# qurAI-amsterdam/SuperResolution_aniso_MRI

Measured on AMD Instinct MI355X. Metric: training slices/sec (ae_combined, 160x160, latent=128), higher is better.
Workload: dtype f32; 1 GPU; ACDC synthetic 12x(3x1x160x160) triplets, ae_combined latent=128 depth=32 scales=2, MSE synthesis loss (BASELINE configs[1]); global_batch_triplets=12, parallelism=dp1, init=reference Initializer, seed 892372, random weights, launch=captured HIP graph replay

## Files before the change

### superresolution_aniso_mri_amd/csrc/conv_wgrad_wino.hip

```cpp
#include <stdio.h>
#include <stdlib.h>

#include <type_traits>
#include <utility>

#include "aesr_kernels.h"

constexpr int WW_OOB = 0x70000000;
typedef float f32x2 __attribute__((ext_vector_type(2)));

template <int... I, class F>
__device__ __forceinline__ void ww_for(std::integer_sequence<int, I...>, F&& f) {
    (f(std::integral_constant<int, I>{}), ...);
}
template <int N, class F>
__device__ __forceinline__ void ww_rep(F&& f) { ww_for(std::make_integer_sequence<int, N>{}, f); }

__device__ __forceinline__ void ww_dma(__amdgpu_buffer_rsrc_t rs, float* lds_wave_base, int byte_off) {
    __builtin_amdgcn_raw_ptr_buffer_load_lds(rs, (__attribute__((address_space(3))) void*)lds_wave_base, 16, byte_off, 0, 0, 0);
}

#define WW_PK(dst, a, b, mods)                                                          \
    do {                                                                                \
        f32x2& d_ = dst;                                                                \
        const f32x2 a_ = a, b_ = b;                                                     \
        asm volatile("v_pk_add_f32 %0, %1, %2 " mods : "=v"(d_) : "v"(a_), "v"(b_));    \
    } while (0)
#define WW_M_ADD ""
#define WW_M_SUB "neg_lo:[0,1] neg_hi:[0,1]"
#define WW_M_T01 "op_sel:[0,0] op_sel_hi:[1,0] neg_lo:[0,1] neg_hi:[0,0]"
#define WW_M_T23 "op_sel:[1,0] op_sel_hi:[1,1] neg_lo:[1,0] neg_hi:[0,1]"
#define WW_M_LL "op_sel:[0,0] op_sel_hi:[0,0] neg_lo:[0,0] neg_hi:[0,1]"
#define WW_M_HH "op_sel:[1,1] op_sel_hi:[1,1] neg_lo:[0,0] neg_hi:[0,1]"
#define WW_M_SELF "op_sel:[0,1] op_sel_hi:[0,1] neg_lo:[0,0] neg_hi:[0,1]"

struct WwTile {
    int n, ty, tx;
};

template <int TH, int TW, bool STAMP>
__global__ __launch_bounds__(256, 1) void conv_wgrad_wino_f32(WgradArgs a) {
    constexpr int CIT = 32, COT = 32;
    static_assert((TH == 16 && TW == 8) || (TH == 8 && TW == 16), "tiles: 8 k-steps, rows of whole 8-pixel DMA segments");
    constexpr int PH = TH + 2, PWL = TW == 8 ? 16 : 32, TWL = TW;
    constexpr int XFL = PH * PWL * 32, DFL = TH * TWL * 32;
    constexpr int KPR = TW >> 3;
    constexpr int SPR = PWL / 8, SPRD = TW / 8;
    constexpr int NXS = PH * SPR / 4, NDS = TH * SPRD / 4;
    constexpr int RXS = 4 / SPR, RDS = 4 / SPRD;
    static_assert(2 * (XFL + DFL) * 4 <= 160 * 1024 && (PH * SPR) % 4 == 0 && (TH * SPRD) % 4 == 0, "LDS / segment split");

    extern __shared__ __attribute__((aligned(16))) float lds[];
    const int tid = threadIdx.x, lane = tid & 63;
    const int wave = __builtin_amdgcn_readfirstlane(tid >> 6);
    const int l15 = lane & 15, g = lane >> 4;
    const int nci = a.CinP / CIT, nchunks = nci * (a.CoutP / COT);
    int chunk, split;
    if ((a.S & 7) == 0) {
        const int xcd = blockIdx.x & 7, local = blockIdx.x >> 3;
        chunk = local % nchunks;
        split = (local / nchunks) * 8 + xcd;
    } else {
        chunk = blockIdx.x % nchunks;
        split = blockIdx.x / nchunks;
    }
    const int ciy = chunk % nci, coz = chunk / nci;
    const int ci0 = ciy * CIT, co0 = coz * COT;
    float* const ldsX0 = lds;
    float* const ldsD0 = lds + 2 * XFL;
    const bool do_bias = ciy == 0;

    const int sh = a.x_up2 ? 1 : 0;
    const int xH = a.H >> sh, xW = a.W >> sh;
    const int ximg = xH * xW * a.Cin * 4, dimg = a.H * a.W * a.Cout * 4;
    const int xrow = xW * a.Cin * 4, drow = a.W * a.Cout * 4;
    const int sgx = wave % SPR, rx0 = wave / SPR, sgd = wave % SPRD, rd0 = wave / SPRD;
    const int pxl = lane >> 3, pos = lane & 7;
    const int quad = pos ^ (((pxl >> 1) & 1) << 2);
    const int pcx = 8 * sgx + pxl, pcd = 8 * sgd + pxl;
    const int lcx = (((pcx - sh) >> sh) * a.Cin + ci0 + 4 * quad) * 4;
    const int lcd = (pcd * a.Cout + co0 + 4 * quad) * 4;
    const int tpi = a.tiles_y * a.tiles_x;
    const int dS_n = a.S / tpi, dS_r = a.S - dS_n * tpi, dS_ty = dS_r / a.tiles_x, dS_tx = dS_r - dS_ty * a.tiles_x;
    auto advance = [&](WwTile t) {
        t.tx += dS_tx;
        if (t.tx >= a.tiles_x) { t.tx -= a.tiles_x; ++t.ty; }
        t.ty += dS_ty;
        if (t.ty >= a.tiles_y) { t.ty -= a.tiles_y; ++t.n; }
        t.n += dS_n;
        return t;
    };
    auto fetch = [&](const WwTile& t, int buf) {
        const bool valid = t.n < a.N;
        const int n = valid ? t.n : 0, y0 = t.ty * TH, x0 = t.tx * TW;
        const __amdgpu_buffer_rsrc_t rs_x = __builtin_amdgcn_make_buffer_rsrc((void*)((const char*)a.x + (size_t)n * ximg), 0, valid ? ximg : 0, 0x00020000);
        const __amdgpu_buffer_rsrc_t rs_d = __builtin_amdgcn_make_buffer_rsrc((void*)((const char*)a.dy + (size_t)n * dimg), 0, valid ? dimg : 0, 0x00020000);
        const unsigned gxx = (unsigned)(x0 - 1 + pcx), gxd = (unsigned)(x0 + pcd);
        const int offx = (pcx < TW + 2 && gxx < (unsigned)a.W) ? lcx + ((x0 >> sh) - 1 + sh) * a.Cin * 4 : WW_OOB;
        const int offd = gxd < (unsigned)a.W ? lcd + x0 * a.Cout * 4 : WW_OOB;
        const int r0 = y0 - 1 + rx0;
        int ux = (r0 >> sh) * xrow;
        const int step_odd = sh == 0 ? RXS * xrow : RXS == 2 ? xrow : (r0 & 1) * xrow;
        const int step_even = sh == 0 ? RXS * xrow : RXS == 2 ? xrow : xrow - step_odd;
        float* const xdst = ldsX0 + buf * XFL + (rx0 * PWL + 8 * sgx) * 32;
        int uxk[NXS];
        ww_rep<NXS>([&](auto Kc) {
            constexpr int k = decltype(Kc)::value;
            if constexpr (k > 0) ux += (k & 1) ? step_odd : step_even;
            uxk[k] = ux;
        });
        if (pcx < TW + 2) {
            ww_rep<NXS>([&](auto Kc) {
                constexpr int k = decltype(Kc)::value;
                ww_dma(rs_x, xdst + k * RXS * PWL * 32, offx + uxk[k]);
            });
        }
        int ud = (y0 + rd0) * drow;
        float* const ddst = ldsD0 + buf * DFL + (rd0 * TWL + 8 * sgd) * 32;
        ww_rep<NDS>([&](auto Kc) {
            constexpr int k = decltype(Kc)::value;
            if constexpr (k > 0) ud += RDS * drow;
            ww_dma(rs_d, ddst + k * RDS * TWL * 32, offd + ud);
        });
    };

    f32x4 acc[16][2][2];
#pragma unroll
    for (int x = 0; x < 16; ++x)
#pragma unroll
        for (int i = 0; i < 2; ++i)
#pragma unroll
            for (int o = 0; o < 2; ++o) acc[x][i][o] = (f32x4){0.f, 0.f, 0.f, 0.f};
    float accb[2] = {0.f, 0.f};

    const int sw = (g & 1) << 2;
    const int chA = (((l15 >> 2) ^ sw) << 2) + (l15 & 3);
    const int chB = (((l15 >> 2) ^ sw ^ 4) << 2) + (l15 & 3);
    const unsigned lds0 = (unsigned)(unsigned long long)lds;
    unsigned lx[2][4], ld[2][2];
#pragma unroll
    for (int i = 0; i < 2; ++i) {
#pragma unroll
        for (int c = 0; c < 4; ++c) lx[i][c] = lds0 + (unsigned)(((2 * g + c) * 32 + ((c < 2 ? chA : chB) ^ (i ? 16 : 0))) * 4);
#pragma unroll
        for (int e = 0; e < 2; ++e) ld[i][e] = lds0 + (unsigned)((2 * XFL + (2 * g + e) * 32 + (chA ^ (i ? 16 : 0))) * 4);
    }

    f32x2 Vp[2][2][2][4], Mp[2][2][8];
    f32x2 P[2][4][2];
    auto op_read = [&](int xu, int du, int nb) {
        ww_rep<8>([&](auto Kc) {
            constexpr int i = decltype(Kc)::value >> 2, c = decltype(Kc)::value & 3;
            const unsigned ad = lx[i][c] + (unsigned)(xu * 4);
            f32x2 &p0_ = P[i][c][0], &p1_ = P[i][c][1];
            asm volatile("ds_read2st64_b32 %0, %2 offset0:%3 offset1:%4\n\tds_read2st64_b32 %1, %2 offset0:%5 offset1:%6"
                         : "=&v"(p0_), "=&v"(p1_) : "v"(ad), "n"(0), "n"(PWL / 2), "n"(PWL), "n"(3 * PWL / 2) : "memory");
        });
        ww_rep<4>([&](auto Kc) {
            constexpr int o = decltype(Kc)::value >> 1, e = decltype(Kc)::value & 1;
            const unsigned ad = ld[o][e] + (unsigned)(du * 4);
            f32x2& y_ = Mp[nb][o][e];
            asm volatile("ds_read2st64_b32 %0, %1 offset0:0 offset1:%2" : "=&v"(y_) : "v"(ad), "n"(TWL / 2) : "memory");
        });
    };
    auto op_transform = [&](int nb) {
        asm volatile("s_waitcnt lgkmcnt(0)" ::: "memory");
        ww_rep<2>([&](auto Ic) {
            constexpr int i = decltype(Ic)::value;
            f32x2 T[2][4];
            ww_rep<4>([&](auto Cc) {
                constexpr int c = decltype(Cc)::value;
                WW_PK(T[0][c], P[i][c][0], P[i][c][1], WW_M_T01);
                WW_PK(T[1][c], P[i][c][0], P[i][c][1], WW_M_T23);
            });
            ww_rep<2>([&](auto Sc) {
                constexpr int s_ = decltype(Sc)::value;
                WW_PK(Vp[nb][i][s_][0], T[s_][0], T[s_][2], WW_M_SUB);
                WW_PK(Vp[nb][i][s_][1], T[s_][1], T[s_][2], WW_M_ADD);
                WW_PK(Vp[nb][i][s_][2], T[s_][2], T[s_][1], WW_M_SUB);
                WW_PK(Vp[nb][i][s_][3], T[s_][1], T[s_][3], WW_M_SUB);
            });
        });
        ww_rep<2>([&](auto Oc) {
            constexpr int o = decltype(Oc)::value;
            WW_PK(Mp[nb][o][2], Mp[nb][o][0], Mp[nb][o][0], WW_M_SELF);
            WW_PK(Mp[nb][o][3], Mp[nb][o][1], Mp[nb][o][1], WW_M_SELF);
            WW_PK(Mp[nb][o][4], Mp[nb][o][0], Mp[nb][o][1], WW_M_LL);
            WW_PK(Mp[nb][o][7], Mp[nb][o][0], Mp[nb][o][1], WW_M_HH);
            WW_PK(Mp[nb][o][5], Mp[nb][o][2], Mp[nb][o][3], WW_M_LL);
            WW_PK(Mp[nb][o][6], Mp[nb][o][2], Mp[nb][o][3], WW_M_HH);
            accb[o] += Mp[nb][o][5][0];
        });
    };
    auto mfmas = [&](auto Q0c, auto Nc, int cb) {
        ww_rep<decltype(Nc)::value>([&](auto Dc) {
            constexpr int q = decltype(Q0c)::value + decltype(Dc)::value, x = q >> 2, i = (q >> 1) & 1, o = q & 1;
            constexpr int r = x >> 2, k = x & 3;
            constexpr int mi = k == 0 ? (r == 0 || r == 3 ? 0 : 2) : k == 3 ? (r == 0 || r == 3 ? 1 : 3) : 4 + r;
            constexpr int mh = k == 0 || k == 3 ? (r >= 2 ? 1 : 0) : k - 1;
            f32x4& acc_ = acc[x][i][o];
            const float va_ = Vp[cb][i][r >> 1][k][r & 1], vb_ = Mp[cb][o][mi][mh];
            asm volatile("v_mfma_f32_16x16x4_f32 %0, %1, %2, %0" : "+a"(acc_) : "v"(va_), "v"(vb_));
        });
    };
    auto step_xu = [&](int j, int buf) { const int ks = wave + 4 * j, tyl = ks / KPR, kx = ks - tyl * KPR; return buf * XFL + ((2 * tyl) * PWL + 8 * kx) * 32; };
    auto step_du = [&](int j, int buf) { const int ks = wave + 4 * j, tyl = ks / KPR, kx = ks - tyl * KPR; return buf * DFL + ((2 * tyl) * TWL + 8 * kx) * 32; };
    using C0 = std::integral_constant<int, 0>;
    using C16 = std::integral_constant<int, 16>;
    using C32 = std::integral_constant<int, 32>;

    long long tph[3] = {0, 0, 0}, tq = 0;
#define WW_STAMP(k)                                                   \
    if constexpr (STAMP) {                                            \
        const long long t_ = (long long)__builtin_amdgcn_s_memtime(); \
        tph[k] += t_ - tq;                                            \
        tq = t_;                                                      \
    }
    if constexpr (STAMP) tq = (long long)__builtin_amdgcn_s_memtime();

    WwTile t0, t1, t2;
    {
        t0.n = split / tpi;
        const int rem = split - t0.n * tpi;
        t0.ty = rem / a.tiles_x;
        t0.tx = rem - t0.ty * a.tiles_x;
        if (split >= a.ntiles) t0.n = a.N;
    }
    t1 = advance(t0);
    t2 = advance(t1);
    fetch(t0, 0);
    fetch(t1, 1);
    asm volatile("s_waitcnt vmcnt(0)" ::: "memory");
    __syncthreads();
    int buf = 0;
    op_read(step_xu(0, 0), step_du(0, 0), 0);
    op_transform(0);
    WW_STAMP(2)
    if (t0.n < a.N) do {
        __builtin_amdgcn_sched_barrier(0);
        op_read(step_xu(1, buf), step_du(1, buf), 1);
        mfmas(C0{}, C16{}, 0);
        op_transform(1);
        mfmas(C16{}, std::integral_constant<int, 48>{}, 0);
        __builtin_amdgcn_sched_barrier(0);
        WW_STAMP(0)
        asm volatile("s_waitcnt vmcnt(0) lgkmcnt(0)" ::: "memory");
        __syncthreads();
        WW_STAMP(1)
        __builtin_amdgcn_sched_barrier(0);
        op_read(step_xu(0, buf ^ 1), step_du(0, buf ^ 1), 0);
        mfmas(C0{}, C16{}, 1);
        __builtin_amdgcn_sched_barrier(0);
        fetch(t2, buf);
        __builtin_amdgcn_sched_barrier(0);
        mfmas(C16{}, C16{}, 1);
        op_transform(0);
        mfmas(C32{}, C32{}, 1);
        __builtin_amdgcn_sched_barrier(0);
        t0 = t1;
        t1 = t2;
        t2 = advance(t2);
        buf ^= 1;
    } while (t0.n < a.N);
    WW_STAMP(0)
    asm volatile("s_waitcnt vmcnt(0) lgkmcnt(0)" ::: "memory");
    __syncthreads();
    if (STAMP && lane == 0)
        for (int k = 0; k < 3; ++k) a.dbgbuf[(blockIdx.x * 4 + wave) * 3 + k] = (float)tph[k];

    f32x4 dg[9][2][2];
#pragma unroll
    for (int i = 0; i < 2; ++i)
#pragma unroll
        for (int o = 0; o < 2; ++o) {
            f32x4 R[3][4];
#pragma unroll
            for (int j = 0; j < 4; ++j) {
                const f32x4 u0_ = acc[0 + j][i][o], u1 = acc[4 + j][i][o], u2 = acc[8 + j][i][o], u3 = -acc[12 + j][i][o];
                const f32x4 s = j == 3 ? (f32x4){-1.f, -1.f, -1.f, -1.f} : (f32x4){1.f, 1.f, 1.f, 1.f};
                R[0][j] = s * (u0_ + 0.5f * (u1 + u2));
                R[1][j] = s * (0.5f * (u1 - u2));
                R[2][j] = s * (0.5f * (u1 + u2) + u3);
            }
#pragma unroll
            for (int r = 0; r < 3; ++r) {
                dg[r * 3 + 0][i][o] = R[r][0] + 0.5f * (R[r][1] + R[r][2]);
                dg[r * 3 + 1][i][o] = 0.5f * (R[r][1] - R[r][2]);
                dg[r * 3 + 2][i][o] = 0.5f * (R[r][1] + R[r][2]) + R[r][3];
            }
        }
#pragma unroll
    for (int o = 0; o < 2; ++o) {
        accb[o] += __shfl_xor(accb[o], 16, 64);
        accb[o] += __shfl_xor(accb[o], 32, 64);
    }
    f32x4* ex = (f32x4*)lds;
    float* exb = lds + 4 * 36 * 64 * 4;
#pragma unroll
    for (int t = 0; t < 9; ++t)
#pragma unroll
        for (int i = 0; i < 2; ++i)
#pragma unroll
            for (int o = 0; o < 2; ++o) ex[(wave * 36 + (t * 4 + i * 2 + o)) * 64 + lane] = dg[t][i][o];
    if (g == 0) {
        exb[wave * 32 + l15] = accb[0];
        exb[wave * 32 + 16 + l15] = accb[1];
    }
    __syncthreads();
    const size_t plane = (size_t)a.CinP * a.CoutP;
    float* sl = a.slab + (size_t)split * 10 * plane;
#pragma unroll
    for (int q = 0; q < 9; ++q) {
        const int blk = wave * 9 + q;
        const int t = blk >> 2, i = (blk >> 1) & 1, o = blk & 1;
        f32x4 v = ex[(0 * 36 + blk) * 64 + lane];
#pragma unroll
        for (int w = 1; w < 4; ++w) v += ex[(w * 36 + blk) * 64 + lane];
        const int co = co0 + o * 16 + l15;
#pragma unroll
        for (int e = 0; e < 4; ++e) {
            const int ci = ci0 + i * 16 + g * 4 + e;
            sl[t * plane + (size_t)ci * a.CoutP + co] = v[e];
        }
    }
    if (wave == 0 && do_bias && g == 0) {
#pragma unroll
        for (int o = 0; o < 2; ++o) {
            float bsum = exb[0 * 32 + o * 16 + l15];
#pragma unroll
            for (int w = 1; w < 4; ++w) bsum += exb[w * 32 + o * 16 + l15];
            sl[9 * plane + co0 + o * 16 + l15] = bsum;
        }
    }
}

size_t aesr_wgrad_wino_lds_bytes(int TH, int TW) {
    const size_t xfl = (size_t)(TH + 2) * (TW == 8 ? 16 : 32) * 32, dfl = (size_t)TH * TW * 32;
    const size_t bufs = 2 * (xfl + dfl) * sizeof(float);
    const size_t exch = ((size_t)4 * 36 * 64 * 4 + 4 * 32) * sizeof(float);
    return bufs > exch ? bufs : exch;
}

bool aesr_wgrad_wino_tile_ok(int TH, int TW) { return (TH == 16 && TW == 8) || (TH == 8 && TW == 16); }

template <int TH, int TW>
static int launch_wgrad_wino(const WgradArgs& a, hipStream_t st) {
    const size_t shmem = aesr_wgrad_wino_lds_bytes(TH, TW);
    static bool attr_set[AESR_MAX_DEVICES] = {}, attr_set_dbg[AESR_MAX_DEVICES] = {};
    if (int e = aesr_lds_opt_in((const void*)conv_wgrad_wino_f32<TH, TW, false>, "conv_wgrad_wino_f32", attr_set)) return e;
    (void)aesr_lds_opt_in((const void*)conv_wgrad_wino_f32<TH, TW, true>, "conv_wgrad_wino_f32", attr_set_dbg);
    dim3 grid(a.S * (a.CinP / 32) * (a.CoutP / 32));
    if (getenv("AESR_WGRAD_WINO_DBG") && grid.x <= 4096) {
        static float* dbuf = nullptr;
        if (!dbuf) (void)hipMalloc(&dbuf, 4096 * 4 * 3 * sizeof(float));
        WgradArgs b = a;
        b.dbgbuf = dbuf;
        hipLaunchKernelGGL((conv_wgrad_wino_f32<TH, TW, true>), grid, dim3(256), shmem, st, b);
        (void)hipStreamSynchronize(st);
        static float host[4096 * 4 * 3];
        (void)hipMemcpy(host, dbuf, (size_t)grid.x * 4 * 3 * sizeof(float), hipMemcpyDeviceToHost);
        double s3[3] = {0, 0, 0};
        for (unsigned i = 0; i < grid.x * 4; ++i) for (int k = 0; k < 3; ++k) s3[k] += host[i * 3 + k];
        const double visits = (double)((a.ntiles + a.S - 1) / a.S);
        const int nks = (TH >> 1) * (TW >> 3);
        fprintf(stderr, "[wgrad-wino stamps] grid=%u tile %dx%d S=%d (%.0f visits, %d k-steps = %d MFMA cycles per wave and visit) per visit, cycles: "
                "k-step loop %.0f | barrier %.0f || fill %.0f\n", grid.x, TH, TW, a.S, visits, nks, nks / 4 * 64 * 32,
                s3[0] / grid.x / 4 / visits, s3[1] / grid.x / 4 / visits, s3[2] / grid.x / 4);
        return AESR_OK;
    }
    hipLaunchKernelGGL((conv_wgrad_wino_f32<TH, TW, false>), grid, dim3(256), shmem, st, a);
    AESR_LAUNCH_CHECK("conv_wgrad_wino_f32");
    return AESR_OK;
}

int aesr_launch_conv_wgrad_wino(const WgradArgs& a, hipStream_t st) {
    if ((size_t)a.H * a.W * a.Cin * 4 >= (size_t)0x10000000 || (size_t)a.H * a.W * a.Cout * 4 >= (size_t)0x10000000) {
        aesr_set_error("conv_wgrad_wino: images of 256 MB or more need 64-bit lane offsets (not built)");
        return AESR_ERR_UNSUPPORTED;
    }
    if (a.x_up2 && ((a.H | a.W) & 1)) {
        aesr_set_error("conv_wgrad_wino: the folded Upsample(x2) needs even convolution sizes (got %dx%d)", a.H, a.W);
        return AESR_ERR_ARG;
    }
    if (!aesr_wgrad_wino_tile_ok(a.TH, a.TW) || a.pad != 1 || a.Ho != a.H || a.Wo != a.W) {
        aesr_set_error("conv_wgrad_wino: tile %dx%d is not 16x8 or 8x16 (or not 3x3 / padding 1)", a.TH, a.TW);
        return AESR_ERR_ARG;
    }
    if (a.CinP % 32 != 0 || a.CoutP % 32 != 0 || a.Cin != a.CinP || a.Cout != a.CoutP || a.S < 1 || a.S > a.ntiles ||
        a.tiles_y != ceil_div(a.H, a.TH) || a.tiles_x != ceil_div(a.W, a.TW) || a.ntiles != a.N * a.tiles_y * a.tiles_x) {
        aesr_set_error("conv_wgrad_wino: channel counts must be multiples of 32 and the tile grid consistent (S=%d, %d tiles)", a.S, a.ntiles);
        return AESR_ERR_ARG;
    }
    if (a.TH == 16) return launch_wgrad_wino<16, 8>(a, st);
    return launch_wgrad_wino<8, 16>(a, st);
}
```

Before: 16310 slices/s.

## Add lean prologue/epilogue to Winograd wgrad kernel with vectorized slab stores

```diff
diff --git a/superresolution_aniso_mri_amd/csrc/conv_wgrad_wino.hip b/superresolution_aniso_mri_amd/csrc/conv_wgrad_wino.hip
--- a/superresolution_aniso_mri_amd/csrc/conv_wgrad_wino.hip
+++ b/superresolution_aniso_mri_amd/csrc/conv_wgrad_wino.hip
@@ -34,11 +34,22 @@
 #define WW_M_HH "op_sel:[1,1] op_sel_hi:[1,1] neg_lo:[0,0] neg_hi:[0,1]"
 #define WW_M_SELF "op_sel:[0,1] op_sel_hi:[0,1] neg_lo:[0,0] neg_hi:[0,1]"
 
+__device__ __forceinline__ f32x4 ww_sub4(f32x4 a, f32x4 b) {
+    f32x2 lo, hi;
+    const f32x2 alo = a.xy, ahi = a.zw, blo = b.xy, bhi = b.zw;
+    asm("v_pk_add_f32 %0, %1, %2 " WW_M_SUB : "=v"(lo) : "v"(alo), "v"(blo));
+    asm("v_pk_add_f32 %0, %1, %2 " WW_M_SUB : "=v"(hi) : "v"(ahi), "v"(bhi));
+    return (f32x4){lo.x, lo.y, hi.x, hi.y};
+}
+typedef float f32x4u __attribute__((ext_vector_type(4), aligned(4)));
+
 struct WwTile {
     int n, ty, tx;
 };
 
-template <int TH, int TW, bool STAMP>
+constexpr int WW_NTS = 10;
+constexpr int WW_DBG_WAVES = 4096 * 4;
+template <int TH, int TW, bool STAMP, bool LEAN>
 __global__ __launch_bounds__(256, 1) void conv_wgrad_wino_f32(WgradArgs a) {
     constexpr int CIT = 32, COT = 32;
     static_assert((TH == 16 && TW == 8) || (TH == 8 && TW == 16), "tiles: 8 k-steps, rows of whole 8-pixel DMA segments");
@@ -51,6 +62,14 @@
     static_assert(2 * (XFL + DFL) * 4 <= 160 * 1024 && (PH * SPR) % 4 == 0 && (TH * SPRD) % 4 == 0, "LDS / segment split");
 
     extern __shared__ __attribute__((aligned(16))) float lds[];
+    unsigned long long ts[WW_NTS] = {};
+#define WW_TS(k)                                          \
+    if constexpr (STAMP) {                                \
+        __builtin_amdgcn_sched_barrier(0);                \
+        ts[k] = __builtin_amdgcn_s_memrealtime();         \
+        __builtin_amdgcn_sched_barrier(0);                \
+    }
+    WW_TS(0)
     const int tid = threadIdx.x, lane = tid & 63;
     const int wave = __builtin_amdgcn_readfirstlane(tid >> 6);
     const int l15 = lane & 15, g = lane >> 4;
@@ -125,12 +144,14 @@
     };
 
     f32x4 acc[16][2][2];
-#pragma unroll
-    for (int x = 0; x < 16; ++x)
-#pragma unroll
-        for (int i = 0; i < 2; ++i)
-#pragma unroll
-            for (int o = 0; o < 2; ++o) acc[x][i][o] = (f32x4){0.f, 0.f, 0.f, 0.f};
+    if constexpr (!LEAN) {
+#pragma unroll
+        for (int x = 0; x < 16; ++x)
+#pragma unroll
+            for (int i = 0; i < 2; ++i)
+#pragma unroll
+                for (int o = 0; o < 2; ++o) acc[x][i][o] = (f32x4){0.f, 0.f, 0.f, 0.f};
+    }
     float accb[2] = {0.f, 0.f};
 
     const int sw = (g & 1) << 2;
@@ -230,12 +251,29 @@
     t2 = advance(t1);
     fetch(t0, 0);
     fetch(t1, 1);
-    asm volatile("s_waitcnt vmcnt(0)" ::: "memory");
-    __syncthreads();
+    WW_TS(1)
+    if constexpr (LEAN) {
+        __builtin_amdgcn_sched_barrier(0);
+        ww_rep<64>([&](auto Qc) {
+            constexpr int q = decltype(Qc)::value;
+            f32x4& acc_ = acc[q >> 2][(q >> 1) & 1][q & 1];
+            acc_ = (f32x4){0.f, 0.f, 0.f, 0.f};
+            asm volatile("" : "+a"(acc_));
+        });
+        __builtin_amdgcn_sched_barrier(0);
+        if (8 * sgx < TW + 2) asm volatile("s_waitcnt vmcnt(%0)" ::"n"(NXS + NDS) : "memory");
+        else asm volatile("s_waitcnt vmcnt(%0)" ::"n"(NDS) : "memory");
+        __builtin_amdgcn_s_barrier();
+    } else {
+        asm volatile("s_waitcnt vmcnt(0)" ::: "memory");
+        __syncthreads();
+    }
+    WW_TS(2)
     int buf = 0;
     op_read(step_xu(0, 0), step_du(0, 0), 0);
     op_transform(0);
     WW_STAMP(2)
+    WW_TS(3)
     if (t0.n < a.N) do {
         __builtin_amdgcn_sched_barrier(0);
         op_read(step_xu(1, buf), step_du(1, buf), 1);
@@ -263,73 +301,152 @@
         buf ^= 1;
     } while (t0.n < a.N);
     WW_STAMP(0)
+    WW_TS(4)
     asm volatile("s_waitcnt vmcnt(0) lgkmcnt(0)" ::: "memory");
     __syncthreads();
+    WW_TS(5)
     if (STAMP && lane == 0)
         for (int k = 0; k < 3; ++k) a.dbgbuf[(blockIdx.x * 4 + wave) * 3 + k] = (float)tph[k];
 
-    f32x4 dg[9][2][2];
-#pragma unroll
-    for (int i = 0; i < 2; ++i)
+    if constexpr (!LEAN) {
+        f32x4 dg[9][2][2];
+#pragma unroll
+        for (int i = 0; i < 2; ++i)
+#pragma unroll
+            for (int o = 0; o < 2; ++o) {
+                f32x4 R[3][4];
+#pragma unroll
+                for (int j = 0; j < 4; ++j) {
+                    const f32x4 u0_ = acc[0 + j][i][o], u1 = acc[4 + j][i][o], u2 = acc[8 + j][i][o], u3 = -acc[12 + j][i][o];
+                    const f32x4 s = j == 3 ? (f32x4){-1.f, -1.f, -1.f, -1.f} : (f32x4){1.f, 1.f, 1.f, 1.f};
+                    R[0][j] = s * (u0_ + 0.5f * (u1 + u2));
+                    R[1][j] = s * (0.5f * (u1 - u2));
+                    R[2][j] = s * (0.5f * (u1 + u2) + u3);
+                }
+#pragma unroll
+                for (int r = 0; r < 3; ++r) {
+                    dg[r * 3 + 0][i][o] = R[r][0] + 0.5f * (R[r][1] + R[r][2]);
+                    dg[r * 3 + 1][i][o] = 0.5f * (R[r][1] - R[r][2]);
+                    dg[r * 3 + 2][i][o] = 0.5f * (R[r][1] + R[r][2]) + R[r][3];
+                }
+            }
 #pragma unroll
         for (int o = 0; o < 2; ++o) {
+            accb[o] += __shfl_xor(accb[o], 16, 64);
+            accb[o] += __shfl_xor(accb[o], 32, 64);
+        }
+        WW_TS(6)
+        f32x4* ex = (f32x4*)lds;
+        float* exb = lds + 4 * 36 * 64 * 4;
+#pragma unroll
+        for (int t = 0; t < 9; ++t)
+#pragma unroll
+            for (int i = 0; i < 2; ++i)
+#pragma unroll
+                for (int o = 0; o < 2; ++o) ex[(wave * 36 + (t * 4 + i * 2 + o)) * 64 + lane] = dg[t][i][o];
+        if (g == 0) {
+            exb[wave * 32 + l15] = accb[0];
+            exb[wave * 32 + 16 + l15] = accb[1];
+        }
+        __syncthreads();
+        WW_TS(7)
+        const size_t plane = (size_t)a.CinP * a.CoutP;
+        float* sl = a.slab + (size_t)split * 10 * plane;
+#pragma unroll
+        for (int q = 0; q < 9; ++q) {
+            const int blk = wave * 9 + q;
+            const int t = blk >> 2, i = (blk >> 1) & 1, o = blk & 1;
+            f32x4 v = ex[(0 * 36 + blk) * 64 + lane];
+#pragma unroll
+            for (int w = 1; w < 4; ++w) v += ex[(w * 36 + blk) * 64 + lane];
+            const int co = co0 + o * 16 + l15;
+#pragma unroll
+            for (int e = 0; e < 4; ++e) {
+                const int ci = ci0 + i * 16 + g * 4 + e;
+                sl[t * plane + (size_t)ci * a.CoutP + co] = v[e];
+            }
+        }
+        if (wave == 0 && do_bias && g == 0) {
+#pragma unroll
+            for (int o = 0; o < 2; ++o) {
+                float bsum = exb[0 * 32 + o * 16 + l15];
+#pragma unroll
+                for (int w = 1; w < 4; ++w) bsum += exb[w * 32 + o * 16 + l15];
+                sl[9 * plane + co0 + o * 16 + l15] = bsum;
+            }
+        }
+    } else {
+        const int ln = (int)__builtin_amdgcn_mbcnt_hi(~0u, __builtin_amdgcn_mbcnt_lo(~0u, 0u));
+        const int e15 = ln & 15, eg = ln >> 4;
+        float* const exf = lds;
+        float* const exb = lds + 4 * 36 * 64 * 4;
+        ww_rep<4>([&](auto Pc) {
+            constexpr int i = decltype(Pc)::value >> 1, o = decltype(Pc)::value & 1;
             f32x4 R[3][4];
-#pragma unroll
-            for (int j = 0; j < 4; ++j) {
-                const f32x4 u0_ = acc[0 + j][i][o], u1 = acc[4 + j][i][o], u2 = acc[8 + j][i][o], u3 = -acc[12 + j][i][o];
-                const f32x4 s = j == 3 ? (f32x4){-1.f, -1.f, -1.f, -1.f} : (f32x4){1.f, 1.f, 1.f, 1.f};
-                R[0][j] = s * (u0_ + 0.5f * (u1 + u2));
-                R[1][j] = s * (0.5f * (u1 - u2));
-                R[2][j] = s * (0.5f * (u1 + u2) + u3);
+            ww_rep<4>([&](auto Jc) {
+                constexpr int j = decltype(Jc)::value;
+                const f32x4 u0_ = acc[0 + j][i][o], u1 = acc[4 + j][i][o], u2 = acc[8 + j][i][o], u3n = acc[12 + j][i][o];
+                const f32x4 h = 0.5f * (u1 + u2);
+                R[0][j] = u0_ + h;
+                R[1][j] = 0.5f * ww_sub4(u1, u2);
+                R[2][j] = ww_sub4(h, u3n);
+            });
+            ww_rep<3>([&](auto Rc) {
+                constexpr int r = decltype(Rc)::value;
+                const f32x4 h = 0.5f * (R[r][1] + R[r][2]);
+                const f32x4 d[3] = {R[r][0] + h, 0.5f * ww_sub4(R[r][1], R[r][2]), ww_sub4(h, R[r][3])};
+                ww_rep<3>([&](auto Cc) {
+                    constexpr int c = decltype(Cc)::value, blk = (r * 3 + c) * 4 + i * 2 + o;
+                    float* const p = exf + (wave * 36 + blk) * 256 + ln;
+#pragma unroll
+                    for (int e = 0; e < 4; ++e) p[e * 64] = d[c][e];
+                });
+            });
+        });
+#pragma unroll
+        for (int o = 0; o < 2; ++o) {
+            accb[o] += __shfl_xor(accb[o], 16, 64);
+            accb[o] += __shfl_xor(accb[o], 32, 64);
+        }
+        if (eg == 0) {
+            exb[wave * 32 + e15] = accb[0];
+            exb[wave * 32 + 16 + e15] = accb[1];
+        }
+        WW_TS(6)
+        __syncthreads();
+        WW_TS(7)
+        const size_t plane = (size_t)a.CinP * a.CoutP;
+        float* sl = a.slab + (size_t)split * 10 * plane;
+        const int rci = ln >> 2, rco = (ln & 3) * 4;
+        const float* const rd = exf + (rci & 3) * 64 + (rci >> 2) * 16 + rco;
+        const unsigned off = (unsigned)(rci * a.CoutP + rco) * 4u, plane4 = (unsigned)plane * 4u;
+#pragma unroll
+        for (int q = 0; q < 9; ++q) {
+            const int blk = wave * 9 + q;
+            const int t = blk >> 2, i = (blk >> 1) & 1, o = blk & 1;
+            f32x4 v = *(const f32x4*)(rd + (0 * 36 + blk) * 256);
+#pragma unroll
+            for (int w = 1; w < 4; ++w) v += *(const f32x4*)(rd + (w * 36 + blk) * 256);
+            const unsigned ub = (unsigned)t * plane4 + (unsigned)((ci0 + i * 16) * a.CoutP + co0 + o * 16) * 4u;
+            *(f32x4u*)((char*)sl + (size_t)(ub + off)) = v;
+        }
+        if (wave == 0 && do_bias && eg == 0) {
+#pragma unroll
+            for (int o = 0; o < 2; ++o) {
+                float bsum = exb[0 * 32 + o * 16 + e15];
+#pragma unroll
+                for (int w = 1; w < 4; ++w) bsum += exb[w * 32 + o * 16 + e15];
+                sl[9 * plane + co0 + o * 16 + e15] = bsum;
             }
-#pragma unroll
-            for (int r = 0; r < 3; ++r) {
-                dg[r * 3 + 0][i][o] = R[r][0] + 0.5f * (R[r][1] + R[r][2]);
-                dg[r * 3 + 1][i][o] = 0.5f * (R[r][1] - R[r][2]);
-                dg[r * 3 + 2][i][o] = 0.5f * (R[r][1] + R[r][2]) + R[r][3];
-            }
-        }
-#pragma unroll
-    for (int o = 0; o < 2; ++o) {
-        accb[o] += __shfl_xor(accb[o], 16, 64);
-        accb[o] += __shfl_xor(accb[o], 32, 64);
-    }
-    f32x4* ex = (f32x4*)lds;
-    float* exb = lds + 4 * 36 * 64 * 4;
-#pragma unroll
-    for (int t = 0; t < 9; ++t)
-#pragma unroll
-        for (int i = 0; i < 2; ++i)
-#pragma unroll
-            for (int o = 0; o < 2; ++o) ex[(wave * 36 + (t * 4 + i * 2 + o)) * 64 + lane] = dg[t][i][o];
-    if (g == 0) {
-        exb[wave * 32 + l15] = accb[0];
-        exb[wave * 32 + 16 + l15] = accb[1];
-    }
-    __syncthreads();
-    const size_t plane = (size_t)a.CinP * a.CoutP;
-    float* sl = a.slab + (size_t)split * 10 * plane;
-#pragma unroll
-    for (int q = 0; q < 9; ++q) {
-        const int blk = wave * 9 + q;
-        const int t = blk >> 2, i = (blk >> 1) & 1, o = blk & 1;
-        f32x4 v = ex[(0 * 36 + blk) * 64 + lane];
-#pragma unroll
-        for (int w = 1; w < 4; ++w) v += ex[(w * 36 + blk) * 64 + lane];
-        const int co = co0 + o * 16 + l15;
-#pragma unroll
-        for (int e = 0; e < 4; ++e) {
-            const int ci = ci0 + i * 16 + g * 4 + e;
-            sl[t * plane + (size_t)ci * a.CoutP + co] = v[e];
-        }
-    }
-    if (wave == 0 && do_bias && g == 0) {
-#pragma unroll
-        for (int o = 0; o < 2; ++o) {
-            float bsum = exb[0 * 32 + o * 16 + l15];
-#pragma unroll
-            for (int w = 1; w < 4; ++w) bsum += exb[w * 32 + o * 16 + l15];
-            sl[9 * plane + co0 + o * 16 + l15] = bsum;
+        }
+    }
+    if constexpr (STAMP) {
+        WW_TS(8)
+        asm volatile("s_waitcnt vmcnt(0)" ::: "memory");
+        WW_TS(9)
+        if (lane == 0) {
+            unsigned long long* out = (unsigned long long*)(a.dbgbuf + WW_DBG_WAVES * 3) + (size_t)(blockIdx.x * 4 + wave) * WW_NTS;
+            for (int k = 0; k < WW_NTS; ++k) out[k] = ts[k];
         }
     }
 }
@@ -343,32 +460,54 @@
 
 bool aesr_wgrad_wino_tile_ok(int TH, int TW) { return (TH == 16 && TW == 8) || (TH == 8 && TW == 16); }
 
-template <int TH, int TW>
+template <int TH, int TW, bool LEAN>
 static int launch_wgrad_wino(const WgradArgs& a, hipStream_t st) {
     const size_t shmem = aesr_wgrad_wino_lds_bytes(TH, TW);
     static bool attr_set[AESR_MAX_DEVICES] = {}, attr_set_dbg[AESR_MAX_DEVICES] = {};
-    if (int e = aesr_lds_opt_in((const void*)conv_wgrad_wino_f32<TH, TW, false>, "conv_wgrad_wino_f32", attr_set)) return e;
-    (void)aesr_lds_opt_in((const void*)conv_wgrad_wino_f32<TH, TW, true>, "conv_wgrad_wino_f32", attr_set_dbg);
+    if (int e = aesr_lds_opt_in((const void*)conv_wgrad_wino_f32<TH, TW, false, LEAN>, "conv_wgrad_wino_f32", attr_set)) return e;
+    (void)aesr_lds_opt_in((const void*)conv_wgrad_wino_f32<TH, TW, true, LEAN>, "conv_wgrad_wino_f32", attr_set_dbg);
     dim3 grid(a.S * (a.CinP / 32) * (a.CoutP / 32));
-    if (getenv("AESR_WGRAD_WINO_DBG") && grid.x <= 4096) {
+    if (getenv("AESR_WGRAD_WINO_DBG") && grid.x * 4 <= (unsigned)WW_DBG_WAVES) {
+        constexpr size_t dbytes = (size_t)WW_DBG_WAVES * (3 * sizeof(float) + WW_NTS * sizeof(unsigned long long));
         static float* dbuf = nullptr;
-        if (!dbuf) (void)hipMalloc(&dbuf, 4096 * 4 * 3 * sizeof(float));
+        if (!dbuf) (void)hipMalloc(&dbuf, dbytes);
         WgradArgs b = a;
         b.dbgbuf = dbuf;
-        hipLaunchKernelGGL((conv_wgrad_wino_f32<TH, TW, true>), grid, dim3(256), shmem, st, b);
+        hipLaunchKernelGGL((conv_wgrad_wino_f32<TH, TW, true, LEAN>), grid, dim3(256), shmem, st, b);
         (void)hipStreamSynchronize(st);
-        static float host[4096 * 4 * 3];
-        (void)hipMemcpy(host, dbuf, (size_t)grid.x * 4 * 3 * sizeof(float), hipMemcpyDeviceToHost);
+        static float host[dbytes / sizeof(float)];
+        (void)hipMemcpy(host, dbuf, dbytes, hipMemcpyDeviceToHost);
+        const unsigned nw = grid.x * 4;
         double s3[3] = {0, 0, 0};
-        for (unsigned i = 0; i < grid.x * 4; ++i) for (int k = 0; k < 3; ++k) s3[k] += host[i * 3 + k];
+        for (unsigned i = 0; i < nw; ++i) for (int k = 0; k < 3; ++k) s3[k] += host[i * 3 + k];
         const double visits = (double)((a.ntiles + a.S - 1) / a.S);
         const int nks = (TH >> 1) * (TW >> 3);
-        fprintf(stderr, "[wgrad-wino stamps] grid=%u tile %dx%d S=%d (%.0f visits, %d k-steps = %d MFMA cycles per wave and visit) per visit, cycles: "
-                "k-step loop %.0f | barrier %.0f || fill %.0f\n", grid.x, TH, TW, a.S, visits, nks, nks / 4 * 64 * 32,
+        fprintf(stderr, "[wgrad-wino stamps] grid=%u tile %dx%d S=%d lean=%d (%.0f visits, %d k-steps = %d MFMA cycles per wave and visit) per visit, cycles: "
+                "k-step loop %.0f | barrier %.0f || fill %.0f\n", grid.x, TH, TW, a.S, (int)LEAN, visits, nks, nks / 4 * 64 * 32,
                 s3[0] / grid.x / 4 / visits, s3[1] / grid.x / 4 / visits, s3[2] / grid.x / 4);
+        const unsigned long long* ts = (const unsigned long long*)(host + WW_DBG_WAVES * 3);
+        unsigned long long first = ~0ull, last = 0;
+        for (unsigned i = 0; i < nw; ++i) {
+            if (ts[(size_t)i * WW_NTS] < first) first = ts[(size_t)i * WW_NTS];
+            if (ts[(size_t)i * WW_NTS + WW_NTS - 1] > last) last = ts[(size_t)i * WW_NTS + WW_NTS - 1];
+        }
+        double ph[WW_NTS] = {}, skew = 0, skew_max = 0;
+        for (unsigned i = 0; i < nw; ++i) {
+            const unsigned long long* t = ts + (size_t)i * WW_NTS;
+            const double e = (double)(t[0] - first) * 0.01;
+            skew += e;
+            if (e > skew_max) skew_max = e;
+            for (int k = 1; k < WW_NTS; ++k) ph[k] += (double)(t[k] - t[k - 1]) * 0.01;
+        }
+        for (int k = 1; k < WW_NTS; ++k) ph[k] /= nw;
+        fprintf(stderr, "[wgrad-wino life] %d->%d N=%d %dx%d lean=%d: span %.2f us | per wave, us: entry behind first wave %.2f (max %.2f) | DMA issue %.2f | "
+                "tile wait+barrier %.2f | first operands %.2f | loop %.2f (%.2f per visit) | drain wait+barrier %.2f | dg %.2f | exchange+barrier %.2f | "
+                "slab stores issued %.2f | stores retired %.2f || outside the loop %.2f\n", a.Cin, a.Cout, a.N, a.H, a.W, (int)LEAN,
+                (double)(last - first) * 0.01, skew / nw, skew_max, ph[1], ph[2], ph[3], ph[4], ph[4] / visits, ph[5], ph[6], ph[7], ph[8], ph[9],
+                ph[1] + ph[2] + ph[3] + ph[5] + ph[6] + ph[7] + ph[8] + ph[9]);
         return AESR_OK;
     }
-    hipLaunchKernelGGL((conv_wgrad_wino_f32<TH, TW, false>), grid, dim3(256), shmem, st, a);
+    hipLaunchKernelGGL((conv_wgrad_wino_f32<TH, TW, false, LEAN>), grid, dim3(256), shmem, st, a);
     AESR_LAUNCH_CHECK("conv_wgrad_wino_f32");
     return AESR_OK;
 }
@@ -391,6 +530,8 @@
         aesr_set_error("conv_wgrad_wino: channel counts must be multiples of 32 and the tile grid consistent (S=%d, %d tiles)", a.S, a.ntiles);
         return AESR_ERR_ARG;
     }
-    if (a.TH == 16) return launch_wgrad_wino<16, 8>(a, st);
-    return launch_wgrad_wino<8, 16>(a, st);
-}
+    static const bool lean_env = [] { const char* e = getenv("AESR_WGRAD_WINO_LEAN"); return !(e && *e && atoi(e) == 0); }();
+    const bool lean = lean_env && (size_t)a.CinP * a.CoutP * 40 < ((size_t)1 << 32);
+    if (a.TH == 16) return lean ? launch_wgrad_wino<16, 8, true>(a, st) : launch_wgrad_wino<16, 8, false>(a, st);
+    return lean ? launch_wgrad_wino<8, 16, true>(a, st) : launch_wgrad_wino<8, 16, false>(a, st);
+}
```

Measured after the change: 16490 slices/s, median of 6. +1.1%, better.
